# evfro/polara

Measured on NVIDIA H100. Metric: user-item pairs scored/sec (fused top-k) at rank 50, higher is better.
Workload: dtype f32 (bf16 tensor-core filter, exact fp32 rescoring)

## Files before the change

polara_b200/csrc/topk_tc.cu:

```cuda
#include <cuda_bf16.h>
#include <cfloat>
#include <cstdlib>
#include <cub/device/device_radix_sort.cuh>

#include "topk_common.cuh"

namespace {

constexpr int BM = 128;
constexpr int BN = 128;
constexpr int NCONS = 256;
constexpr int NTHREADS = NCONS + 32;
constexpr int CAPS = 16;
constexpr int MAX_STAGES = 10;
constexpr uint32_t STAGE_BYTES = BN * 128;
constexpr int PROBE_ITEMS = 256;
constexpr int HEAD_TILES = 8;
constexpr int HEAD_WORDS = HEAD_TILES * BN / 32;
constexpr long long SPIN_LIMIT_CYCLES = 4000000000ll;

struct TcParams {
    const __nv_bfloat16* Ap;
    const __nv_bfloat16* Bp;
    const float* E; int64_t lde;
// ... 161 lines not shown
    int64_t total = user_tiles * BM * chunks;
    if (gid >= total) return;
    int64_t tile = gid / ((int64_t)BM * chunks);
    int rem = (int)(gid % ((int64_t)BM * chunks));
    int row = rem / chunks, ch = rem % chunks;
    const int64_t tr = tile * BM + row;
    const int64_t u = (tr < m && uperm) ? (int64_t)__ldg(uperm + tr) : tr;
    __align__(16) __nv_bfloat16 out[8];
    uint32_t thr = 0;
    if (ch == rs / 8) {
        if (u < m) {
            thr = pack_threshold(t0[u]);
        } else {
            thr = 0x00007F7Fu;
        }
    }
#pragma unroll
    for (int j = 0; j < 8; ++j) {
        int kk = ch * 8 + j;
        float x = 0.f;
        if (u < m && kk < r) x = -__ldg(E + u * lde + kk);
        out[j] = __float2bfloat16_rn(x);
        if (kk == rs) out[j] = __ushort_as_bfloat16((unsigned short)(thr & 0xFFFFu));
        if (kk == rs + 1) out[j] = __ushort_as_bfloat16((unsigned short)(thr >> 16));
        if (kk == rs + 2 && u < m)
            out[j] = __ushort_as_bfloat16((unsigned short)(0x8000u | bf16_ceil_pos_bits(0.0079345703125f * enorm[u] + 1e-30f)));
    }
    size_t byte = (size_t)tile * BM * chunks * 16 + tile_byte(BM, row, ch * 8);
    *reinterpret_cast<uint4*>(reinterpret_cast<unsigned char*>(Ap) + byte) = *reinterpret_cast<const uint4*>(out);
}

__global__ void row_norm_kernel(const float* __restrict__ X, int64_t ld, int64_t rows, int r, float* __restrict__ norms,
                                float* __restrict__ max_out) {
    int64_t w = ((int64_t)blockIdx.x * blockDim.x + threadIdx.x) >> 5;
    int lane = threadIdx.x & 31;
    if (w >= rows) return;
    float s = 0.f;
    for (int t = lane; t < r; t += 32) { float x = __ldg(X + w * ld + t); s = fmaf(x, x, s); }
#pragma unroll
    for (int o = 16; o > 0; o >>= 1) s += __shfl_xor_sync(0xffffffffu, s, o);
    s = sqrtf(s) * 1.0001f;
    if (lane == 0) {
        if (norms) norms[w] = s;
        if (max_out) atomicMax(reinterpret_cast<int*>(max_out), __float_as_int(s));
    }
}

__global__ void iota_i32_kernel(int32_t* __restrict__ x, int64_t n) {
    int64_t i = (int64_t)blockIdx.x * blockDim.x + threadIdx.x;
    if (i < n) x[i] = (int32_t)i;
}

__global__ void invert_perm_kernel(const int32_t* __restrict__ perm, int64_t n, int32_t* __restrict__ inv) {
    int64_t i = (int64_t)blockIdx.x * blockDim.x + threadIdx.x;
    if (i < n) inv[perm[i]] = (int32_t)i;
}

__global__ void head_items_kernel(const int32_t* __restrict__ perm, int64_t n_head, uint32_t* __restrict__ in_head) {
    int64_t i = (int64_t)blockIdx.x * blockDim.x + threadIdx.x;
    if (i < n_head) { const int32_t item = perm[i]; atomicOr(in_head + (item >> 5), 1u << (item & 31)); }
}

__global__ void __launch_bounds__(256)
head_bitmap_kernel(const int64_t* __restrict__ seen_indptr, const int32_t* __restrict__ seen_indices,
                   int64_t seen_offset, const int32_t* __restrict__ inv_perm, const uint32_t* __restrict__ in_head,
                   int64_t m, int64_t n, uint32_t* __restrict__ bits) {
    static_assert(HEAD_WORDS == 32, "one bitmap word per lane");
    __shared__ uint32_t sw[8][HEAD_WORDS];
    const int64_t u = ((int64_t)blockIdx.x * blockDim.x + threadIdx.x) >> 5;
    const int lane = threadIdx.x & 31, warp = threadIdx.x >> 5;
    if (u >= m) return;
    sw[warp][lane] = 0u;
    __syncwarp();
    for (int64_t p = seen_indptr[u] + lane; p < seen_indptr[u + 1]; p += 32) {
        int64_t item = (int64_t)__ldg(seen_indices + p) - seen_offset;
        if (item < 0 || item >= n) continue;
        if (!((__ldg(in_head + (item >> 5)) >> (item & 31)) & 1u)) continue;
        int pos = __ldg(inv_perm + item);
        atomicOr(&sw[warp][pos >> 5], 0x80000000u >> (pos & 31));
    }
    __syncwarp();
    bits[u * HEAD_WORDS + lane] = sw[warp][lane];
}

__device__ __forceinline__ int first_cut_tile(float en, float t, const float* __restrict__ vnorm_sorted, int lo, int hi) {
    if (!(t > 0.f && t < CUDART_INF_F)) return hi;
    while (lo < hi) {
        const int mid = (lo + hi) >> 1;
        if (en * __ldg(vnorm_sorted + (int64_t)mid * BN) < t) hi = mid; else lo = mid + 1;
    }
    return lo;
}

__global__ void user_need_kernel(const float* __restrict__ enorm, const float* __restrict__ t0,
                                 const float* __restrict__ vnorm_sorted, int64_t m, int item_tiles, int32_t* __restrict__ need) {
    const int64_t u = (int64_t)blockIdx.x * blockDim.x + threadIdx.x;
    if (u < m) need[u] = first_cut_tile(__ldg(enorm + u), __ldg(t0 + u), vnorm_sorted, 0, item_tiles);
}

constexpr int PTU = 64, PTI = 128, PKS = 32;
constexpr int PNU = 2;
template <int PI>
struct ProbeSmem {
    float es[PKS][PTU + 4];
    float vs[PKS][PTI + 4];
    float sc[PTU][PI + 4];
    unsigned long long cand[8][PNU][32];
    float t0s[PTU];
};

__device__ __forceinline__ uint32_t ord_of(float x) {
    const uint32_t b = __float_as_uint(x);
    return (b & 0x80000000u) ? ~b : (b | 0x80000000u);
}
__device__ __forceinline__ float ord_to_float(uint32_t o) {
    return __uint_as_float((o & 0x80000000u) ? (o & 0x7FFFFFFFu) : ~o);
}

template <int PL>
__device__ __noinline__ void probe_select_rounds(unsigned long long (&key)[PL], int lane, int k,
                                                 pb200_cand* __restrict__ out, float* __restrict__ t0_u) {
    static_assert(PL == 8, "the sorting network below is for 8 keys per lane");
#define PB_CAS(A, B) { const unsigned long long x_ = key[A], y_ = key[B]; const bool g_ = x_ > y_; key[A] = g_ ? x_ : y_; key[B] = g_ ? y_ : x_; }
    PB_CAS(0, 1) PB_CAS(2, 3) PB_CAS(4, 5) PB_CAS(6, 7)
    PB_CAS(0, 2) PB_CAS(1, 3) PB_CAS(4, 6) PB_CAS(5, 7)
    PB_CAS(1, 2) PB_CAS(5, 6)
    PB_CAS(0, 4) PB_CAS(1, 5) PB_CAS(2, 6) PB_CAS(3, 7)
    PB_CAS(2, 4) PB_CAS(3, 5)
    PB_CAS(1, 2) PB_CAS(3, 4) PB_CAS(5, 6)
#undef PB_CAS
    float kth = -CUDART_INF_F;
    int produced = 0;
    pb200_cand mine; mine.score = -CUDART_INF_F; mine.id = -1;
    for (; produced < k; ++produced) {
        const uint32_t hh = (uint32_t)(key[0] >> 32), hl = (uint32_t)key[0];
        const uint32_t wh = __reduce_max_sync(0xffffffffu, hh);
        if (wh == 0u) break;
        const uint32_t wl = __reduce_max_sync(0xffffffffu, hh == wh ? hl : 0u);
        if (hh == wh && hl == wl) {
#pragma unroll
            for (int j = 0; j + 1 < PL; ++j) key[j] = key[j + 1];
            key[PL - 1] = 0ull;
        }
        const float ws = ord_to_float(wh);
        if (lane == (produced & 31)) { mine.score = ws; mine.id = (int)(0xFFFFFFFFu - wl); }
        if ((produced & 31) == 31) out[(produced - 31) + lane] = mine;
        kth = ws;
    }
    if (lane < (produced & 31)) out[(produced & ~31) + lane] = mine;
    for (int j = produced + lane; j < k; j += 32) { pb200_cand c; c.score = -CUDART_INF_F; c.id = -1; out[j] = c; }
    if (lane == 0) *t0_u = produced == k ? kth : -CUDART_INF_F;
}

template <int PI>
__global__ void __launch_bounds__(256)
probe_kernel(const float* __restrict__ E, int64_t lde, const float* __restrict__ V, int64_t ldv,
             const int32_t* __restrict__ perm, int64_t m, int64_t n_probe, int r, int k,
             const uint32_t* __restrict__ headbits, float* __restrict__ t0, pb200_cand* __restrict__ out_list,
             float* __restrict__ enorm, const float* __restrict__ vnorm_sorted, int item_tiles, int32_t* __restrict__ need) {
    extern __shared__ __align__(16) unsigned char praw[];
    ProbeSmem<PI>& sm = *reinterpret_cast<ProbeSmem<PI>*>(praw);
    const int tid = threadIdx.x, lane = tid & 31, warp = tid >> 5, tx = tid & 15, ty = tid >> 4;
    const int64_t u0 = (int64_t)blockIdx.x * PTU;
    const bool vec = ((lde | ldv) & 3) == 0 && ((reinterpret_cast<uintptr_t>(E) | reinterpret_cast<uintptr_t>(V)) & 15) == 0;
    const int n_ktiles = (r + PKS - 1) / PKS, n_tiles = (PI / PTI) * n_ktiles;
    const int64_t eu = u0 + (tid & (PTU - 1));
    const float* erow = eu < m ? E + eu * lde : nullptr;
    const float* vrow = nullptr;
    float4 pe[2], pv[4];
    auto fetch = [&](int tile) {
        const int i0 = (tile / n_ktiles) * PTI, k0 = (tile % n_ktiles) * PKS;
        if (tile % n_ktiles == 0) {
            const int64_t vpos = i0 + (tid & (PTI - 1));
            vrow = vpos < n_probe ? V + (int64_t)__ldg(perm + vpos) * ldv : nullptr;
        }
#pragma unroll
        for (int it = 0; it < 2; ++it) {
            const int kq = k0 + 4 * ((tid >> 6) + 4 * it);
            pe[it] = (erow && kq < r) ? __ldg(reinterpret_cast<const float4*>(erow + kq)) : make_float4(0.f, 0.f, 0.f, 0.f);
        }
#pragma unroll
        for (int it = 0; it < 4; ++it) {
            const int kq = k0 + 4 * ((tid >> 7) + 2 * it);
            pv[it] = (vrow && kq < r) ? __ldg(reinterpret_cast<const float4*>(vrow + kq)) : make_float4(0.f, 0.f, 0.f, 0.f);
        }
    };
    auto stash = [&](int tile) {
        const int k0 = (tile % n_ktiles) * PKS;
#pragma unroll
        for (int it = 0; it < 2; ++it) {
            const int q = (tid >> 6) + 4 * it, kq = k0 + 4 * q, row = tid & (PTU - 1);
            sm.es[4 * q + 0][row] = pe[it].x;
            sm.es[4 * q + 1][row] = kq + 1 < r ? pe[it].y : 0.f;
            sm.es[4 * q + 2][row] = kq + 2 < r ? pe[it].z : 0.f;
            sm.es[4 * q + 3][row] = kq + 3 < r ? pe[it].w : 0.f;
        }
#pragma unroll
        for (int it = 0; it < 4; ++it) {
            const int q = (tid >> 7) + 2 * it, kq = k0 + 4 * q, row = tid & (PTI - 1);
            sm.vs[4 * q + 0][row] = pv[it].x;
            sm.vs[4 * q + 1][row] = kq + 1 < r ? pv[it].y : 0.f;
            sm.vs[4 * q + 2][row] = kq + 2 < r ? pv[it].z : 0.f;
            sm.vs[4 * q + 3][row] = kq + 3 < r ? pv[it].w : 0.f;
        }
    };
    if (vec) fetch(0);
    float acc[4][8];
    float en2 = 0.f;
    for (int tile = 0; tile < n_tiles; ++tile) {
        const int i0 = (tile / n_ktiles) * PTI, k0 = (tile % n_ktiles) * PKS;
        if (k0 == 0) {
#pragma unroll
            for (int a = 0; a < 4; ++a)
#pragma unroll
                for (int b = 0; b < 8; ++b) acc[a][b] = 0.f;
        }
        if (vec) {
            stash(tile);
        } else {
#pragma unroll
            for (int it = 0; it < 8; ++it) {
                int e = tid + it * 256, row = e >> 5, kk = e & 31;
                int64_t u = u0 + row;
                sm.es[kk][row] = (u < m && k0 + kk < r) ? __ldg(E + u * lde + k0 + kk) : 0.f;
            }
#pragma unroll
            for (int it = 0; it < 16; ++it) {
                int e = tid + it * 256, row = e >> 5, kk = e & 31;
                int64_t pos = i0 + row;
                sm.vs[kk][row] = (pos < n_probe && k0 + kk < r) ? __ldg(V + (int64_t)__ldg(perm + pos) * ldv + k0 + kk) : 0.f;
            }
        }
        __syncthreads();
        if (vec && tile + 1 < n_tiles) fetch(tile + 1);
        const int kmax = min(PKS, r - k0);
        if (i0 == 0 && tid < PTU)
            for (int kk = 0; kk < kmax; ++kk) en2 = fmaf(sm.es[kk][tid], sm.es[kk][tid], en2);
        for (int kk = 0; kk < kmax; ++kk) {
            float4 e4 = *reinterpret_cast<const float4*>(&sm.es[kk][ty * 4]);
            float4 v0 = *reinterpret_cast<const float4*>(&sm.vs[kk][tx * 4]);
            float4 v1 = *reinterpret_cast<const float4*>(&sm.vs[kk][64 + tx * 4]);
            float a[4] = {e4.x, e4.y, e4.z, e4.w};
            float b[8] = {v0.x, v0.y, v0.z, v0.w, v1.x, v1.y, v1.z, v1.w};
#pragma unroll
            for (int i = 0; i < 4; ++i)
#pragma unroll
                for (int j = 0; j < 8; ++j) acc[i][j] = fmaf(a[i], b[j], acc[i][j]);
        }
        if (k0 + PKS >= r) {
#pragma unroll
            for (int i = 0; i < 4; ++i)
#pragma unroll
                for (int hseg = 0; hseg < 2; ++hseg) {
                    const int pos = i0 + 64 * hseg + tx * 4;
                    float4 x;
                    x.x = pos + 0 < n_probe ? acc[i][4 * hseg + 0] : -CUDART_INF_F;
                    x.y = pos + 1 < n_probe ? acc[i][4 * hseg + 1] : -CUDART_INF_F;
                    x.z = pos + 2 < n_probe ? acc[i][4 * hseg + 2] : -CUDART_INF_F;
                    x.w = pos + 3 < n_probe ? acc[i][4 * hseg + 3] : -CUDART_INF_F;
                    *reinterpret_cast<float4*>(&sm.sc[ty * 4 + i][pos]) = x;
                }
        }
        __syncthreads();
    }
    constexpr int PL = PI / 32;
    const uint32_t lt_mask = (1u << lane) - 1u;
    for (int ul = warp; ul < PTU; ul += 8 * PNU) {
        int64_t u[PNU];
        bool act[PNU];
        uint32_t seen_w[PNU], ord[PNU][PL], lmax[PNU], tau[PNU];
        int count[PNU] = {};
#pragma unroll
        for (int a = 0; a < PNU; ++a) {
            u[a] = u0 + ul + 8 * a;
            act[a] = ul + 8 * a < PTU && u[a] < m;
            seen_w[a] = 0u;
            if (act[a] && headbits && lane < PL) seen_w[a] = __ldg(headbits + u[a] * HEAD_WORDS + lane);
        }
#pragma unroll
        for (int a = 0; a < PNU; ++a) {
            lmax[a] = 0u;
#pragma unroll
            for (int j = 0; j < PL; ++j) {
                const int pos = lane + 32 * j;
                const uint32_t w = __shfl_sync(0xffffffffu, seen_w[a], j);
                const bool ok = act[a] && pos < n_probe && !(w & (0x80000000u >> lane));
                ord[a][j] = ok ? ord_of(sm.sc[act[a] ? ul + 8 * a : 0][pos] + 0.f) : 0u;
                lmax[a] = max(lmax[a], ord[a][j]);
            }
        }
        const bool small_k = k <= 32;
        if (small_k) {
            uint32_t rest[PNU], w[PNU];
#pragma unroll
            for (int a = 0; a < PNU; ++a) { rest[a] = lmax[a]; w[a] = 0u; }
            for (int i = 0; i < k; ++i) {
#pragma unroll
                for (int a = 0; a < PNU; ++a) {
                    w[a] = __reduce_max_sync(0xffffffffu, rest[a]);
                    if (rest[a] == w[a]) rest[a] = 0u;
                }
            }
#pragma unroll
            for (int a = 0; a < PNU; ++a) tau[a] = w[a] == 0u ? 1u : w[a];
#pragma unroll
            for (int a = 0; a < PNU; ++a) count[a] = 0;
#pragma unroll
            for (int j = 0; j < PL; ++j)
#pragma unroll
                for (int a = 0; a < PNU; ++a) {
                    const bool in = ord[a][j] >= tau[a];
                    const uint32_t b = __ballot_sync(0xffffffffu, in);
                    const int slot = count[a] + __popc(b & lt_mask);
                    if (in && slot < 32) sm.cand[warp][a][slot] = ((unsigned long long)ord[a][j] << 32) | (uint32_t)(lane + 32 * j);
                    count[a] += __popc(b);
                }
        }
        bool fast[PNU];
#pragma unroll
        for (int a = 0; a < PNU; ++a) fast[a] = act[a] && small_k && count[a] <= 32;
        __syncwarp();
        unsigned long long mine[PNU];
        uint32_t mpos[PNU];
#pragma unroll
        for (int a = 0; a < PNU; ++a) {
            mine[a] = 0ull;
            mpos[a] = 0u;
            if (fast[a] && lane < count[a]) {
                const unsigned long long c = sm.cand[warp][a][lane];
                mpos[a] = (uint32_t)c;
                const uint32_t id = (uint32_t)__ldg(perm + (uint32_t)c);
                mine[a] = (c & 0xFFFFFFFF00000000ull) | (unsigned long long)(0xFFFFFFFFu - id);
            }
        }
        __syncwarp();
#pragma unroll
        for (int a = 0; a < PNU; ++a) if (fast[a]) sm.cand[warp][a][lane] = mine[a];
        __syncwarp();
#pragma unroll
        for (int a = 0; a < PNU; ++a) {
            if (!fast[a]) continue;
            pb200_cand* out = out_list + u[a] * k;
            int rank = 0;
            for (int t = 0; t < count[a]; ++t) rank += sm.cand[warp][a][t] > mine[a] ? 1 : 0;
            if (lane < count[a] && rank < k) {
                pb200_cand c; c.score = ord_to_float((uint32_t)(mine[a] >> 32)); c.id = (int)(0xFFFFFFFFu - (uint32_t)mine[a]);
                if (c.score == 0.f) c.score = sm.sc[ul + 8 * a][mpos[a]];
                out[rank] = c;
                if (rank == k - 1) sm.t0s[ul + 8 * a] = c.score;
            }
            if (count[a] < k) {
                if (lane >= count[a] && lane < k) { pb200_cand c; c.score = -CUDART_INF_F; c.id = -1; out[lane] = c; }
                if (lane == 0) sm.t0s[ul + 8 * a] = -CUDART_INF_F;
            }
        }
        __syncwarp();
#pragma unroll
        for (int a = 0; a < PNU; ++a) {
            if (!act[a] || fast[a]) continue;
            unsigned long long key[PL];
#pragma unroll
            for (int j = 0; j < PL; ++j) {
                const uint32_t id = ord[a][j] ? (uint32_t)__ldg(perm + lane + 32 * j) : 0u;
                key[j] = ord[a][j] ? (((unsigned long long)ord[a][j] << 32) | (unsigned long long)(0xFFFFFFFFu - id)) : 0ull;
            }
            probe_select_rounds<PL>(key, lane, k, out_list + u[a] * k, &sm.t0s[ul + 8 * a]);
        }
        __syncwarp();
#pragma unroll
        for (int a = 0; a < PNU; ++a) {
            if (!act[a] || fast[a]) continue;
            pb200_cand* out = out_list + u[a] * k;
            for (int j = lane; j < k; j += 32) {
                const pb200_cand c = out[j];
                if (c.id >= 0 && c.score == 0.f) out[j].score = exact_score(E + u[a] * lde, V + (int64_t)c.id * ldv, r);
            }
        }
    }
    __syncthreads();
    if (tid < PTU && u0 + tid < m) {
        const int64_t uu = u0 + tid;
        const float t = sm.t0s[tid], en = sqrtf(en2) * 1.0001f;
        t0[uu] = t;
        enorm[uu] = en;
        if (need) need[uu] = first_cut_tile(en, t, vnorm_sorted, 0, item_tiles);
    }
}

__device__ __forceinline__ float exact_score_vec(const float* __restrict__ erow, const float* __restrict__ vrow, int r, bool vec_ok) {
    if (!vec_ok) return exact_score(erow, vrow, r);
    const int r4 = r / 4;
    const float4* e4 = reinterpret_cast<const float4*>(erow);
    const float4* v4 = reinterpret_cast<const float4*>(vrow);
    float s = 0.f;
    int t = 0;
    for (; t + 8 <= r4; t += 8) {
        float4 a[8], b[8];
#pragma unroll
        for (int i = 0; i < 8; ++i) { a[i] = __ldg(e4 + t + i); b[i] = __ldg(v4 + t + i); }
#pragma unroll
        for (int i = 0; i < 8; ++i) {
            s = fmaf(a[i].x, b[i].x, s); s = fmaf(a[i].y, b[i].y, s);
            s = fmaf(a[i].z, b[i].z, s); s = fmaf(a[i].w, b[i].w, s);
        }
    }
    for (; t + 4 <= r4; t += 4) {
        float4 a[4], b[4];
#pragma unroll
        for (int i = 0; i < 4; ++i) { a[i] = __ldg(e4 + t + i); b[i] = __ldg(v4 + t + i); }
#pragma unroll
        for (int i = 0; i < 4; ++i) {
            s = fmaf(a[i].x, b[i].x, s); s = fmaf(a[i].y, b[i].y, s);
            s = fmaf(a[i].z, b[i].z, s); s = fmaf(a[i].w, b[i].w, s);
        }
    }
    for (; t < r4; ++t) {
        float4 a = __ldg(e4 + t), b = __ldg(v4 + t);
        s = fmaf(a.x, b.x, s); s = fmaf(a.y, b.y, s); s = fmaf(a.z, b.z, s); s = fmaf(a.w, b.w, s);
    }
    for (int tt = r4 * 4; tt < r; ++tt) s = fmaf(__ldg(erow + tt), __ldg(vrow + tt), s);
    return s;
}

struct ListState {
    pb200_cand* list;
    int cnt;
    float kth;
};

__device__ __forceinline__ void list_insert(ListState& ls, int k, float s, int id) {
    if (ls.cnt == k) {
        pb200_cand last = ls.list[k - 1];
        if (!cand_before(s, id, last.score, last.id)) return;
    }
    int i = ls.cnt < k ? ls.cnt : k - 1;
    while (i > 0) {
        pb200_cand p = ls.list[i - 1];
        if (!cand_before(s, id, p.score, p.id)) break;
        ls.list[i] = p;
        --i;
    }
    pb200_cand c; c.score = s; c.id = id;
    ls.list[i] = c;
    if (ls.cnt < k) ls.cnt++;
    if (ls.cnt == k) ls.kth = ls.list[k - 1].score;
}

constexpr int COOP_MIN = 64;
struct CoopArgs {
    const float* V; int64_t ldv; const int32_t* perm; const int32_t* seen_indices; int64_t seen_offset; int64_t n; int r, k;
};
__device__ __noinline__ int coop_flush_row(const CoopArgs p, const float* __restrict__ erow, const uint2* __restrict__ stage_row,
                                           int n_entries, int64_t t_lo, int64_t sb, int64_t se, bool head_masked,
                                           pb200_cand* __restrict__ list, float t_row, bool vec_ok, int lane, int& cnt, float& kth) {
    int n_scored = 0;
    for (int e = 0; e < n_entries; ++e) {
        const uint2 ent = stage_row[e * 256];
        const int64_t pos = (int64_t)(t_lo + (ent.x >> 2)) * BN + (ent.x & 3) * 32 + lane;
        bool ok = ((ent.y << lane) & 0x80000000u) != 0u && pos < p.n;
        int item = -1;
        float s = 0.f;
        if (ok) {
            item = __ldg(p.perm + pos);
            if (sb < se && (!head_masked || pos >= HEAD_TILES * BN) &&
                seen_lookup(p.seen_indices, sb, se, (int)(item + p.seen_offset))) ok = false;
        }
        if (ok) {
            s = exact_score_vec(erow, p.V + (int64_t)item * p.ldv, p.r, vec_ok);
            ++n_scored;
            ok = !(s < t_row);
        }
        uint32_t pass = __ballot_sync(0xffffffffu, ok);
        while (pass) {
            const int l = __ffs(pass) - 1;
            pass &= pass - 1;
            const float sl = __shfl_sync(0xffffffffu, s, l);
            const int il = __shfl_sync(0xffffffffu, item, l);
            if (sl < t_row) continue;
            cnt = warp_list_insert(list, p.k, cnt, sl, il, lane);
            if (cnt == p.k) { kth = list[p.k - 1].score; t_row = fmaxf(t_row, kth); }
        }
    }
    return n_scored;
}

__global__ void __launch_bounds__(NTHREADS, 1)
score_topk_tc_kernel(const TcParams p) {
    extern __shared__ __align__(1024) unsigned char smem[];
    unsigned char* sA = smem + ((1024u - (smem_u32(smem) & 1023u)) & 1023u);
    unsigned char* sB = sA + p.a_bytes;
    uint2* sStage = reinterpret_cast<uint2*>(sB + (size_t)p.stages * STAGE_BYTES);
    volatile uint2* sThr = reinterpret_cast<volatile uint2*>(sStage + CAPS * 256);
    uint64_t* bars = reinterpret_cast<uint64_t*>(const_cast<uint2*>(sThr) + 256);
    const uint32_t bar_full = smem_u32(bars), bar_empty = smem_u32(bars + MAX_STAGES);
    const uint32_t bar_afull = smem_u32(bars + 2 * MAX_STAGES), bar_aempty = smem_u32(bars + 2 * MAX_STAGES + 1);
    volatile uint32_t* flush_gen = reinterpret_cast<volatile uint32_t*>(bars + 2 * MAX_STAGES + 2);
    volatile unsigned long long* sCut = reinterpret_cast<volatile unsigned long long*>(bars + 2 * MAX_STAGES + 4);
    volatile uint32_t* sStop = reinterpret_cast<volatile uint32_t*>(bars + 2 * MAX_STAGES + 4 + NCONS / 32);

    const int tid = threadIdx.x, warp = tid >> 5, lane = tid & 31;
    if (tid < 256) { const_cast<uint2*>(sThr)[tid] = make_uint2(0u, 0u); }
    if (tid < NCONS / 32) sCut[tid] = 0ull;
    if (tid < MAX_STAGES) sStop[tid] = 0u;
    if (tid == 0) {
        *flush_gen = 0u;
        for (int s = 0; s < p.stages; ++s) { mbar_init(bar_full + 8 * s, 1); mbar_init(bar_empty + 8 * s, NCONS / 32); }
        mbar_init(bar_afull, 1);
        mbar_init(bar_aempty, NCONS / 32);
        fence_barrier_init();
        if (p.hdbg && blockIdx.x == 0) p.hdbg[5] = bar_full;
    }
    __syncthreads();

    const int64_t n_groups = p.user_tiles * p.parts;
    const int64_t n_ctas = gridDim.x, cta = blockIdx.x;
    WorkItem wk;
    const uint32_t S = (uint32_t)p.stages;
    const int KA = (p.KP + 63) / 64;

    if (warp == NCONS / 32) {
        if (lane == 0) {
            uint32_t stage = 0, phase = 0, awork = 0;
            for (int64_t wi = 0; next_work(p, wi, cta, n_ctas, n_groups, wk); ++wi, ++awork) {
                const int64_t t_lo = min(p.item_tiles, p.tile_first + (int64_t)wk.part * p.tiles_per_part);
                int64_t t_hi = min(p.item_tiles, p.tile_first + (int64_t)(wk.part + 1) * p.tiles_per_part);
                if (p.need_sorted) t_hi = min(t_hi, max(t_lo, (int64_t)__ldg(p.need_sorted + wk.g * BM)));
                mbar_wait(bar_aempty, (awork & 1) ^ 1, p.stats, p.hdbg);
                mbar_arrive_expect_tx(bar_afull, p.a_bytes);
                bulk_g2s(smem_u32(sA), reinterpret_cast<const unsigned char*>(p.Ap) + (size_t)wk.g * p.a_bytes, p.a_bytes, bar_afull);
                for (int64_t t = t_lo; t < t_hi; ++t) {
                    if (p.need_sorted) {
                        bool all = true;
                        int64_t live_cut = 0;
#pragma unroll
                        for (int w = 0; w < NCONS / 32; ++w) {
                            const unsigned long long e = sCut[w];
                            all = all && (uint32_t)e == awork + 1;
                            live_cut = max(live_cut, (int64_t)(e >> 32));
// ... 133 lines not shown
                const int64_t t = t_lo + j;
                if (p.need_sorted) {
                    const uint32_t st = gslab % S, ph = (gslab / S) & 1u;
                    mbar_wait(bar_full + 8 * st, ph, p.stats, p.hdbg);
                    if (sStop[st]) {
                        ++gslab;
                        __syncwarp();
                        if (lane == 0) mbar_arrive(bar_empty + 8 * st);
                        break;
                    }
                }
                float d[64];
#pragma unroll
                for (int i = 0; i < 64; ++i) d[i] = 0.f;
                uint32_t prev = 0;
                for (int sl = 0; sl < KA; ++sl) {
                    const uint32_t st = gslab % S, ph = (gslab / S) & 1u;
                    ++gslab;
                    mbar_wait(bar_full + 8 * st, ph, p.stats, p.hdbg);
                    wg_fence_acc(d);
                    wg_fence();
#pragma unroll
                    for (int ks = 0; ks < 4; ++ks)
                        wgmma_m64n128k16(d, adesc0 + (uint64_t)((uint32_t)sl * (BM * 128 / 16) + (uint32_t)ks * 2),
                                         bdesc0 + (uint64_t)(st * (STAGE_BYTES / 16) + (uint32_t)ks * 2), (sl | ks) != 0);
                    wg_commit();
                    wg_fence_acc(d);
                    if (sl > 0) {
                        wg_wait<1>();
                        __syncwarp();
                        if (lane == 0) mbar_arrive(bar_empty + 8 * prev);
                    }
                    prev = st;
                }
                wg_wait<0>();
                wg_fence_acc(d);
                __syncwarp();
                if (lane == 0) mbar_arrive(bar_empty + 8 * prev);

                uint32_t w[2][4];
#pragma unroll
                for (int a = 0; a < 2; ++a)
#pragma unroll
                    for (int c = 0; c < 4; ++c) {
                        uint32_t mk = 0;
#pragma unroll
                        for (int i = 0; i < 4; ++i)
#pragma unroll
                            for (int b = 0; b < 2; ++b)
                                mk |= (__float_as_uint(d[4 * (4 * c + i) + 2 * a + b]) >> 31) << (31 - 8 * i - b);
                        mk >>= 2 * q;
                        mk |= __shfl_xor_sync(0xffffffffu, mk, 1);
                        mk |= __shfl_xor_sync(0xffffffffu, mk, 2);
                        w[a][c] = mk;
                    }
                const bool hi_row = (q >> 1) != 0;
                uint32_t m0 = hi_row ? (h ? w[1][2] : w[1][0]) : (h ? w[0][2] : w[0][0]);
                uint32_t m1 = hi_row ? (h ? w[1][3] : w[1][1]) : (h ? w[0][3] : w[0][1]);
                if (head && t < HEAD_TILES) {
                    const uint2 hb = __ldg(reinterpret_cast<const uint2*>(head + (int)t * (BN / 32) + 2 * h));
                    m0 &= ~hb.x; m1 &= ~hb.y;
                }
                const uint32_t code = (uint32_t)j << 2;
                if (m0 && live) { sStage[scount * 256 + etid] = make_uint2(code | (uint32_t)(2 * h), m0); ++scount; }
                if (m1 && live) { sStage[scount * 256 + etid] = make_uint2(code | (uint32_t)(2 * h + 1), m1); ++scount; }
                {
                    const uint32_t gen = *flush_gen;
                    const bool need = __any_sync(0xffffffffu, scount > CAPS - 2 || (scount >= 4 && t_row == -CUDART_INF_F));
                    if (need || gen != my_gen) {
                        if (need && gen == my_gen && lane == 0) atomicAdd(const_cast<uint32_t*>(flush_gen), 1u);
                        flush();
                        my_gen = *flush_gen;
                        if (p.need_sorted) publish_cut(t + 1);
                    }
                }
            }
            n_swept += (unsigned long long)j;
            flush();
            __syncwarp();
            if (lane == 0) mbar_arrive(bar_aempty);
        }
        if (p.stats && n_rescored) atomicAdd(p.stats + 1, n_rescored);
        if (p.stats && tid == 0 && n_swept) atomicAdd(p.stats + 5, n_swept);
    }
    __syncthreads();
}

}

int pb_score_tc(pb200_ctx* ctx, const float* E, int64_t lde, const float* V, int64_t ldv, int64_t m, int64_t n,
                int r, const int64_t* seen_indptr, const int32_t* seen_indices, int64_t seen_offset, int k,
                int* parts_out, pb200_cand** lists_out, Scratch& sc) {
    const int rs = (r + 1) & ~1;
    const int KP = ((rs + 3) + 15) / 16 * 16;
    const int KA = (KP + 63) / 64;
    const uint32_t a_bytes = BM * KA * 128, b_bytes = BN * KA * 128;
    const size_t fixed = (size_t)a_bytes + CAPS * 256 * sizeof(uint2) + 256 * sizeof(uint2) + (2 * MAX_STAGES + 4) * 8 +
                         (NCONS / 32) * 8 + MAX_STAGES * 4 + 1024;
    int dev_smem = 0;
    PB_CUDA(ctx, cudaDeviceGetAttribute(&dev_smem, cudaDevAttrMaxSharedMemoryPerBlockOptin, ctx->device));
    const int64_t user_tiles = ceil_div64(m, BM), item_tiles = ceil_div64(n, BN);
    const int stages = (int)std::min<int64_t>(MAX_STAGES, ((int64_t)dev_smem - (int64_t)fixed) / STAGE_BYTES);
    if (stages < 2) {
        ctx->err = "tensor-core scoring kernel: rank too large for the shared-memory pipeline (use the simt kernel)";
        return PB200_ENOTIMPL;
    }
    const int64_t n_probe = std::min<int64_t>(PROBE_ITEMS, (n / BN) * BN);
    const int64_t tile_first = n_probe / BN, sweep_tiles = item_tiles - tile_first;
    int parts = (int)std::max<int64_t>(1, std::min<int64_t>(std::min<int64_t>(ceil_div64(2 * (int64_t)ctx->num_sms, user_tiles), 64),
                                                              std::max<int64_t>(sweep_tiles, 1)));
    const int64_t tiles_per_part = std::max<int64_t>(1, ceil_div64(sweep_tiles, parts));
    parts = (int)std::max<int64_t>(1, ceil_div64(sweep_tiles, tiles_per_part));

    __nv_bfloat16 *Ap = nullptr, *Bp = nullptr;
    float *enorm = nullptr, *vnorm = nullptr, *vnorm_sorted = nullptr, *t0 = nullptr;
    int32_t *iota = nullptr, *perm = nullptr, *inv_perm = nullptr;
    uint32_t* headbits = nullptr;
    pb200_cand* lists = nullptr;
    PB_TRY(sc.alloc(&Ap, (size_t)user_tiles * BM * KA * 64));
    PB_TRY(sc.alloc(&Bp, (size_t)item_tiles * BN * KA * 64));
    PB_TRY(sc.alloc(&enorm, (size_t)m));
    PB_TRY(sc.alloc(&vnorm, (size_t)n));
    PB_TRY(sc.alloc(&vnorm_sorted, (size_t)n));
    PB_TRY(sc.alloc(&iota, (size_t)n));
    PB_TRY(sc.alloc(&perm, (size_t)n));
    PB_TRY(sc.alloc(&t0, (size_t)m));
    PB_TRY(sc.alloc(&lists, (size_t)(parts * 2 + 1) * m * k));

    row_norm_kernel<<<(unsigned)ceil_div64(n * 32, 256), 256, 0, ctx->stream>>>(V, ldv, n, r, vnorm, nullptr);
    iota_i32_kernel<<<(unsigned)ceil_div64(n, 256), 256, 0, ctx->stream>>>(iota, n);
    {
        size_t temp_bytes = 0;
        PB_CUDA(ctx, cub::DeviceRadixSort::SortPairsDescending(nullptr, temp_bytes, vnorm, vnorm_sorted, iota, perm, (int64_t)n, 0, 32, ctx->stream));
        uint8_t* temp = nullptr;
        PB_TRY(sc.alloc(&temp, temp_bytes));
        PB_CUDA(ctx, cub::DeviceRadixSort::SortPairsDescending(temp, temp_bytes, vnorm, vnorm_sorted, iota, perm, (int64_t)n, 0, 32, ctx->stream));
    }
    if (seen_indptr) {
        PB_TRY(sc.alloc(&inv_perm, (size_t)n));
        PB_TRY(sc.alloc(&headbits, (size_t)m * HEAD_WORDS));
        invert_perm_kernel<<<(unsigned)ceil_div64(n, 256), 256, 0, ctx->stream>>>(perm, n, inv_perm);
        uint32_t* in_head = nullptr;
        const int64_t n_head = std::min<int64_t>(n, (int64_t)HEAD_TILES * BN);
        PB_TRY(sc.alloc(&in_head, (size_t)ceil_div64(n, 32)));
        PB_CUDA(ctx, cudaMemsetAsync(in_head, 0, (size_t)ceil_div64(n, 32) * sizeof(uint32_t), ctx->stream));
        head_items_kernel<<<(unsigned)ceil_div64(n_head, 256), 256, 0, ctx->stream>>>(perm, n_head, in_head);
        head_bitmap_kernel<<<(unsigned)ceil_div64(m * 32, 256), 256, 0, ctx->stream>>>(seen_indptr, seen_indices, seen_offset,
                                                                                     inv_perm, in_head, m, n, headbits);
    }
    const bool prune = ctx->prune != 0;
    int32_t* need = nullptr;
    if (prune) PB_TRY(sc.alloc(&need, (size_t)m));
    {
        PB_CUDA(ctx, cudaFuncSetAttribute(probe_kernel<PROBE_ITEMS>, cudaFuncAttributeMaxDynamicSharedMemorySize, (int)sizeof(ProbeSmem<PROBE_ITEMS>)));
        probe_kernel<PROBE_ITEMS><<<(unsigned)ceil_div64(m, PTU), 256, sizeof(ProbeSmem<PROBE_ITEMS>), ctx->stream>>>(
            E, lde, V, ldv, perm, m, n_probe, r, k, headbits, t0, lists + (size_t)parts * 2 * m * k,
            enorm, vnorm_sorted, (int)item_tiles, ctx->bound_fn ? nullptr : need);
    }
    if (ctx->bound_fn) {
        const int st = ctx->bound_fn(ctx->bound_user, t0, m, PB200_F32);
        if (st != 0) {
            ctx->err = "bound hook failed with status " + std::to_string(st);
            return PB200_ECUDA;
        }
        if (prune) user_need_kernel<<<(unsigned)ceil_div64(m, 256), 256, 0, ctx->stream>>>(enorm, t0, vnorm_sorted, m, (int)item_tiles, need);
    }
    int32_t *uperm = nullptr, *need_sorted = nullptr;
    if (prune) {
        int32_t* uiota = nullptr;
        PB_TRY(sc.alloc(&uiota, (size_t)m));
        PB_TRY(sc.alloc(&uperm, (size_t)m));
        PB_TRY(sc.alloc(&need_sorted, (size_t)m));
        iota_i32_kernel<<<(unsigned)ceil_div64(m, 256), 256, 0, ctx->stream>>>(uiota, m);
        int end_bit = 1;
        while (end_bit < 31 && ((int64_t)1 << end_bit) <= item_tiles) ++end_bit;
        size_t temp_bytes = 0;
        PB_CUDA(ctx, cub::DeviceRadixSort::SortPairsDescending(nullptr, temp_bytes, need, need_sorted, uiota, uperm, m, 0, end_bit, ctx->stream));
        uint8_t* temp = nullptr;
        PB_TRY(sc.alloc(&temp, temp_bytes));
        PB_CUDA(ctx, cub::DeviceRadixSort::SortPairsDescending(temp, temp_bytes, need, need_sorted, uiota, uperm, m, 0, end_bit, ctx->stream));
    }
    {
        int64_t tot_b = item_tiles * BN * (KA * 8), tot_a = user_tiles * BM * (KA * 8);
        pack_items_kernel<<<(unsigned)ceil_div64(tot_b, 256), 256, 0, ctx->stream>>>(V, ldv, n, r, rs, KP, item_tiles, perm, vnorm_sorted, Bp);
        pack_users_kernel<<<(unsigned)ceil_div64(tot_a, 256), 256, 0, ctx->stream>>>(E, lde, m, r, rs, KP, user_tiles, uperm, enorm, t0, Ap);
    }
    if (sweep_tiles <= 0) {
        cudaEventRecord(ctx->ev0, ctx->stream);
        cudaEventRecord(ctx->ev1, ctx->stream);
        *parts_out = 1;
        *lists_out = lists + (size_t)parts * 2 * m * k;
        PB_CUDA(ctx, cudaGetLastError());
        return PB200_OK;
    }
    TcParams p;
    p.Ap = Ap; p.Bp = Bp; p.E = E; p.lde = lde; p.V = V; p.ldv = ldv; p.perm = perm; p.t0 = t0;
    p.m = m; p.n = n; p.r = r; p.KP = KP; p.rs = rs; p.k = k;
    p.user_tiles = user_tiles; p.item_tiles = item_tiles; p.parts = parts; p.tiles_per_part = tiles_per_part;
    p.tile_first = tile_first;
    p.seen_indptr = seen_indptr; p.seen_indices = seen_indices; p.seen_offset = seen_offset;
    p.lists = lists; p.stages = stages; p.a_bytes = a_bytes; p.b_bytes = b_bytes;
    p.uperm = uperm; p.need_sorted = need_sorted; p.enorm = enorm; p.vnorm_sorted = vnorm_sorted; p.headbits = headbits;
    p.stats = reinterpret_cast<unsigned long long*>(ctx->d_stats);
    p.hdbg = nullptr;
    if (ctx->h_dbg) {
        unsigned long long* dptr = nullptr;
        if (cudaHostGetDevicePointer(&dptr, ctx->h_dbg, 0) == cudaSuccess) p.hdbg = dptr;
    }
    const size_t smem_bytes = fixed + (size_t)stages * STAGE_BYTES;
    PB_CUDA(ctx, cudaFuncSetAttribute(score_topk_tc_kernel, cudaFuncAttributeMaxDynamicSharedMemorySize, (int)smem_bytes));
    const int64_t n_groups = user_tiles * parts;
    const unsigned grid = (unsigned)std::min<int64_t>(n_groups, ctx->num_sms);
    cudaEventRecord(ctx->ev0, ctx->stream);
    score_topk_tc_kernel<<<grid, NTHREADS, smem_bytes, ctx->stream>>>(p);
    cudaEventRecord(ctx->ev1, ctx->stream);
    ctx->stats[0] += (seen_indptr ? 13 : 10) + (prune ? 2 : 0) + (prune && ctx->bound_fn ? 1 : 0);
    ctx->stats[2] = (uint64_t)item_tiles; ctx->stats[3] = (uint64_t)user_tiles;
    ctx->stats[6] += (uint64_t)(user_tiles * sweep_tiles);
    PB_CUDA(ctx, cudaGetLastError());
    *parts_out = parts * 2 + 1;
    *lists_out = lists;
    return PB200_OK;
}
```

Before: 15330 billion.

## Add persistent probe kernel with smem-resident head items and double-buffered user rows

Adds a persistent probe kernel that loads the 256 head items' factor columns into shared memory once per CTA. It then loops over 32-user blocks, prefetching the next block's user rows and seen-bitmap words with cp.async double buffering. The old streamed probe kernel is kept as a fallback when shared memory does not allow two CTAs per SM, and the shared selection logic moves into a templated helper. The aim is to stop re-reading item vectors for every user tile and to hide load latency, at the cost of more shared memory per CTA. The probe is only one stage of the whole top-k pipeline.

```diff
diff --git a/polara_b200/csrc/topk_tc.cu b/polara_b200/csrc/topk_tc.cu
--- a/polara_b200/csrc/topk_tc.cu
+++ b/polara_b200/csrc/topk_tc.cu
@@ -337,9 +337,131 @@
     if (lane == 0) *t0_u = produced == k ? kth : -CUDART_INF_F;
 }
 
+template <int PI, int NU, typename IdOf, typename SeenOf>
+__device__ __forceinline__ void probe_select(const float (*sc)[PI + 4], unsigned long long (*cand)[PNU][32], float* t0s,
+                                             IdOf id_of, bool has_seen, SeenOf seen_word, int64_t u0, int64_t m,
+                                             int64_t n_probe, int k, pb200_cand* __restrict__ out_list,
+                                             const float* __restrict__ E, int64_t lde, const float* __restrict__ V,
+                                             int64_t ldv, int r, int warp, int lane) {
+    constexpr int PL = PI / 32;
+    const uint32_t lt_mask = (1u << lane) - 1u;
+    for (int ul = warp; ul < NU; ul += 8 * PNU) {
+        int64_t u[PNU];
+        bool act[PNU];
+        uint32_t seen_w[PNU], ord[PNU][PL], lmax[PNU], tau[PNU];
+        int count[PNU] = {};
+#pragma unroll
+        for (int a = 0; a < PNU; ++a) {
+            u[a] = u0 + ul + 8 * a;
+            act[a] = ul + 8 * a < NU && u[a] < m;
+            seen_w[a] = 0u;
+            if (act[a] && has_seen && lane < PL) seen_w[a] = seen_word(ul + 8 * a, lane);
+        }
+#pragma unroll
+        for (int a = 0; a < PNU; ++a) {
+            lmax[a] = 0u;
+#pragma unroll
+            for (int j = 0; j < PL; ++j) {
+                const int pos = lane + 32 * j;
+                const uint32_t w = __shfl_sync(0xffffffffu, seen_w[a], j);
+                const bool ok = act[a] && pos < n_probe && !(w & (0x80000000u >> lane));
+                ord[a][j] = ok ? ord_of(sc[act[a] ? ul + 8 * a : 0][pos] + 0.f) : 0u;
+                lmax[a] = max(lmax[a], ord[a][j]);
+            }
+        }
+        const bool small_k = k <= 32;
+        if (small_k) {
+            uint32_t rest[PNU], w[PNU];
+#pragma unroll
+            for (int a = 0; a < PNU; ++a) { rest[a] = lmax[a]; w[a] = 0u; }
+            for (int i = 0; i < k; ++i) {
+#pragma unroll
+                for (int a = 0; a < PNU; ++a) {
+                    w[a] = __reduce_max_sync(0xffffffffu, rest[a]);
+                    if (rest[a] == w[a]) rest[a] = 0u;
+                }
+            }
+#pragma unroll
+            for (int a = 0; a < PNU; ++a) tau[a] = w[a] == 0u ? 1u : w[a];
+#pragma unroll
+            for (int a = 0; a < PNU; ++a) count[a] = 0;
+#pragma unroll
+            for (int j = 0; j < PL; ++j)
+#pragma unroll
+                for (int a = 0; a < PNU; ++a) {
+                    const bool in = ord[a][j] >= tau[a];
+                    const uint32_t b = __ballot_sync(0xffffffffu, in);
+                    const int slot = count[a] + __popc(b & lt_mask);
+                    if (in && slot < 32) cand[warp][a][slot] = ((unsigned long long)ord[a][j] << 32) | (uint32_t)(lane + 32 * j);
+                    count[a] += __popc(b);
+                }
+        }
+        bool fast[PNU];
+#pragma unroll
+        for (int a = 0; a < PNU; ++a) fast[a] = act[a] && small_k && count[a] <= 32;
+        __syncwarp();
+        unsigned long long mine[PNU];
+        uint32_t mpos[PNU];
+#pragma unroll
+        for (int a = 0; a < PNU; ++a) {
+            mine[a] = 0ull;
+            mpos[a] = 0u;
+            if (fast[a] && lane < count[a]) {
+                const unsigned long long c = cand[warp][a][lane];
+                mpos[a] = (uint32_t)c;
+                const uint32_t id = (uint32_t)id_of((uint32_t)c);
+                mine[a] = (c & 0xFFFFFFFF00000000ull) | (unsigned long long)(0xFFFFFFFFu - id);
+            }
+        }
+        __syncwarp();
+#pragma unroll
+        for (int a = 0; a < PNU; ++a) if (fast[a]) cand[warp][a][lane] = mine[a];
+        __syncwarp();
+#pragma unroll
+        for (int a = 0; a < PNU; ++a) {
+            if (!fast[a]) continue;
+            pb200_cand* out = out_list + u[a] * k;
+            int rank = 0;
+            for (int t = 0; t < count[a]; ++t) rank += cand[warp][a][t] > mine[a] ? 1 : 0;
+            if (lane < count[a] && rank < k) {
+                pb200_cand c; c.score = ord_to_float((uint32_t)(mine[a] >> 32)); c.id = (int)(0xFFFFFFFFu - (uint32_t)mine[a]);
+                if (c.score == 0.f) c.score = sc[ul + 8 * a][mpos[a]];
+                out[rank] = c;
+                if (rank == k - 1) t0s[ul + 8 * a] = c.score;
+            }
+            if (count[a] < k) {
+                if (lane >= count[a] && lane < k) { pb200_cand c; c.score = -CUDART_INF_F; c.id = -1; out[lane] = c; }
+                if (lane == 0) t0s[ul + 8 * a] = -CUDART_INF_F;
+            }
+        }
+        __syncwarp();
+#pragma unroll
+        for (int a = 0; a < PNU; ++a) {
+            if (!act[a] || fast[a]) continue;
+            unsigned long long key[PL];
+#pragma unroll
+            for (int j = 0; j < PL; ++j) {
+                const uint32_t id = ord[a][j] ? (uint32_t)id_of(lane + 32 * j) : 0u;
+                key[j] = ord[a][j] ? (((unsigned long long)ord[a][j] << 32) | (unsigned long long)(0xFFFFFFFFu - id)) : 0ull;
+            }
+            probe_select_rounds<PL>(key, lane, k, out_list + u[a] * k, &t0s[ul + 8 * a]);
+        }
+        __syncwarp();
+#pragma unroll
+        for (int a = 0; a < PNU; ++a) {
+            if (!act[a] || fast[a]) continue;
+            pb200_cand* out = out_list + u[a] * k;
+            for (int j = lane; j < k; j += 32) {
+                const pb200_cand c = out[j];
+                if (c.id >= 0 && c.score == 0.f) out[j].score = exact_score(E + u[a] * lde, V + (int64_t)c.id * ldv, r);
+            }
+        }
+    }
+}
+
 template <int PI>
 __global__ void __launch_bounds__(256)
-probe_kernel(const float* __restrict__ E, int64_t lde, const float* __restrict__ V, int64_t ldv,
+probe_streamed_kernel(const float* __restrict__ E, int64_t lde, const float* __restrict__ V, int64_t ldv,
              const int32_t* __restrict__ perm, int64_t m, int64_t n_probe, int r, int k,
              const uint32_t* __restrict__ headbits, float* __restrict__ t0, pb200_cand* __restrict__ out_list,
              float* __restrict__ enorm, const float* __restrict__ vnorm_sorted, int item_tiles, int32_t* __restrict__ need) {
@@ -448,120 +570,9 @@
         }
         __syncthreads();
     }
-    constexpr int PL = PI / 32;
-    const uint32_t lt_mask = (1u << lane) - 1u;
-    for (int ul = warp; ul < PTU; ul += 8 * PNU) {
-        int64_t u[PNU];
-        bool act[PNU];
-        uint32_t seen_w[PNU], ord[PNU][PL], lmax[PNU], tau[PNU];
-        int count[PNU] = {};
-#pragma unroll
-        for (int a = 0; a < PNU; ++a) {
-            u[a] = u0 + ul + 8 * a;
-            act[a] = ul + 8 * a < PTU && u[a] < m;
-            seen_w[a] = 0u;
-            if (act[a] && headbits && lane < PL) seen_w[a] = __ldg(headbits + u[a] * HEAD_WORDS + lane);
-        }
-#pragma unroll
-        for (int a = 0; a < PNU; ++a) {
-            lmax[a] = 0u;
-#pragma unroll
-            for (int j = 0; j < PL; ++j) {
-                const int pos = lane + 32 * j;
-                const uint32_t w = __shfl_sync(0xffffffffu, seen_w[a], j);
-                const bool ok = act[a] && pos < n_probe && !(w & (0x80000000u >> lane));
-                ord[a][j] = ok ? ord_of(sm.sc[act[a] ? ul + 8 * a : 0][pos] + 0.f) : 0u;
-                lmax[a] = max(lmax[a], ord[a][j]);
-            }
-        }
-        const bool small_k = k <= 32;
-        if (small_k) {
-            uint32_t rest[PNU], w[PNU];
-#pragma unroll
-            for (int a = 0; a < PNU; ++a) { rest[a] = lmax[a]; w[a] = 0u; }
-            for (int i = 0; i < k; ++i) {
-#pragma unroll
-                for (int a = 0; a < PNU; ++a) {
-                    w[a] = __reduce_max_sync(0xffffffffu, rest[a]);
-                    if (rest[a] == w[a]) rest[a] = 0u;
-                }
-            }
-#pragma unroll
-            for (int a = 0; a < PNU; ++a) tau[a] = w[a] == 0u ? 1u : w[a];
-#pragma unroll
-            for (int a = 0; a < PNU; ++a) count[a] = 0;
-#pragma unroll
-            for (int j = 0; j < PL; ++j)
-#pragma unroll
-                for (int a = 0; a < PNU; ++a) {
-                    const bool in = ord[a][j] >= tau[a];
-                    const uint32_t b = __ballot_sync(0xffffffffu, in);
-                    const int slot = count[a] + __popc(b & lt_mask);
-                    if (in && slot < 32) sm.cand[warp][a][slot] = ((unsigned long long)ord[a][j] << 32) | (uint32_t)(lane + 32 * j);
-                    count[a] += __popc(b);
-                }
-        }
-        bool fast[PNU];
-#pragma unroll
-        for (int a = 0; a < PNU; ++a) fast[a] = act[a] && small_k && count[a] <= 32;
-        __syncwarp();
-        unsigned long long mine[PNU];
-        uint32_t mpos[PNU];
-#pragma unroll
-        for (int a = 0; a < PNU; ++a) {
-            mine[a] = 0ull;
-            mpos[a] = 0u;
-            if (fast[a] && lane < count[a]) {
-                const unsigned long long c = sm.cand[warp][a][lane];
-                mpos[a] = (uint32_t)c;
-                const uint32_t id = (uint32_t)__ldg(perm + (uint32_t)c);
-                mine[a] = (c & 0xFFFFFFFF00000000ull) | (unsigned long long)(0xFFFFFFFFu - id);
-            }
-        }
-        __syncwarp();
-#pragma unroll
-        for (int a = 0; a < PNU; ++a) if (fast[a]) sm.cand[warp][a][lane] = mine[a];
-        __syncwarp();
-#pragma unroll
-        for (int a = 0; a < PNU; ++a) {
-            if (!fast[a]) continue;
-            pb200_cand* out = out_list + u[a] * k;
-            int rank = 0;
-            for (int t = 0; t < count[a]; ++t) rank += sm.cand[warp][a][t] > mine[a] ? 1 : 0;
-            if (lane < count[a] && rank < k) {
-                pb200_cand c; c.score = ord_to_float((uint32_t)(mine[a] >> 32)); c.id = (int)(0xFFFFFFFFu - (uint32_t)mine[a]);
-                if (c.score == 0.f) c.score = sm.sc[ul + 8 * a][mpos[a]];
-                out[rank] = c;
-                if (rank == k - 1) sm.t0s[ul + 8 * a] = c.score;
-            }
-            if (count[a] < k) {
-                if (lane >= count[a] && lane < k) { pb200_cand c; c.score = -CUDART_INF_F; c.id = -1; out[lane] = c; }
-                if (lane == 0) sm.t0s[ul + 8 * a] = -CUDART_INF_F;
-            }
-        }
-        __syncwarp();
-#pragma unroll
-        for (int a = 0; a < PNU; ++a) {
-            if (!act[a] || fast[a]) continue;
-            unsigned long long key[PL];
-#pragma unroll
-            for (int j = 0; j < PL; ++j) {
-                const uint32_t id = ord[a][j] ? (uint32_t)__ldg(perm + lane + 32 * j) : 0u;
-                key[j] = ord[a][j] ? (((unsigned long long)ord[a][j] << 32) | (unsigned long long)(0xFFFFFFFFu - id)) : 0ull;
-            }
-            probe_select_rounds<PL>(key, lane, k, out_list + u[a] * k, &sm.t0s[ul + 8 * a]);
-        }
-        __syncwarp();
-#pragma unroll
-        for (int a = 0; a < PNU; ++a) {
-            if (!act[a] || fast[a]) continue;
-            pb200_cand* out = out_list + u[a] * k;
-            for (int j = lane; j < k; j += 32) {
-                const pb200_cand c = out[j];
-                if (c.id >= 0 && c.score == 0.f) out[j].score = exact_score(E + u[a] * lde, V + (int64_t)c.id * ldv, r);
-            }
-        }
-    }
+    probe_select<PI, PTU>(sm.sc, sm.cand, sm.t0s, [&](uint32_t pos) { return __ldg(perm + pos); }, headbits != nullptr,
+                          [&](int row, int j) { return __ldg(headbits + (u0 + row) * HEAD_WORDS + j); }, u0, m, n_probe, k,
+                          out_list, E, lde, V, ldv, r, warp, lane);
     __syncthreads();
     if (tid < PTU && u0 + tid < m) {
         const int64_t uu = u0 + tid;
@@ -569,6 +580,152 @@
         t0[uu] = t;
         enorm[uu] = en;
         if (need) need[uu] = first_cut_tile(en, t, vnorm_sorted, 0, item_tiles);
+    }
+}
+
+__device__ __forceinline__ void cp_async4(void* dst, const void* src) {
+    asm volatile("cp.async.ca.shared.global [%0], [%1], 4;" ::"r"(smem_u32(dst)), "l"(src) : "memory");
+}
+__device__ __forceinline__ void cp_async16(void* dst, const void* src) {
+    asm volatile("cp.async.cg.shared.global [%0], [%1], 16;" ::"r"(smem_u32(dst)), "l"(src) : "memory");
+}
+__device__ __forceinline__ void cp_async_commit() { asm volatile("cp.async.commit_group;" ::: "memory"); }
+__device__ __forceinline__ void cp_async_wait1() { asm volatile("cp.async.wait_group 1;" ::: "memory"); }
+
+constexpr int PRU = 32;
+template <int PI>
+struct ProbeResSmem {
+    float sc[PRU][PI + 4];
+    unsigned long long cand[8][PNU][32];
+    float t0s[PRU];
+    int32_t ids[PI];
+    uint32_t hb[2][PRU][PI / 32];
+};
+__host__ __device__ __forceinline__ int probe_res_stride(int r) {
+    const int se = (r + 3) & ~3;
+    return (se & 7) ? se : se + 4;
+}
+template <int PI>
+__host__ __device__ __forceinline__ size_t probe_res_smem_bytes(int r) {
+    return sizeof(ProbeResSmem<PI>) + sizeof(float) * ((size_t)2 * PRU * probe_res_stride(r) + (size_t)r * PI);
+}
+
+template <int PI>
+__global__ void __launch_bounds__(256, 2)
+probe_kernel(const float* __restrict__ E, int64_t lde, const float* __restrict__ V, int64_t ldv,
+             const int32_t* __restrict__ perm, int64_t m, int64_t n_probe, int r, int k,
+             const uint32_t* __restrict__ headbits, float* __restrict__ t0, pb200_cand* __restrict__ out_list,
+             float* __restrict__ enorm, const float* __restrict__ vnorm_sorted, int item_tiles, int32_t* __restrict__ need) {
+    static_assert(PI == 256, "one head item per thread in the load, two 128-item halves in the product");
+    extern __shared__ __align__(16) unsigned char praw[];
+    ProbeResSmem<PI>& sm = *reinterpret_cast<ProbeResSmem<PI>*>(praw);
+    const int SE = probe_res_stride(r);
+    float* const es = reinterpret_cast<float*>(praw + sizeof(ProbeResSmem<PI>));
+    float* const vs = es + 2 * PRU * SE;
+    const int tid = threadIdx.x, lane = tid & 31, warp = tid >> 5;
+    const bool vec = (lde & 3) == 0 && (reinterpret_cast<uintptr_t>(E) & 15) == 0;
+    const int64_t n_blocks = (m + PRU - 1) / PRU;
+    auto load_e = [&](int64_t b, int buf) {
+        float* dst = es + buf * PRU * SE;
+        const int64_t ub = b * PRU;
+        if (vec) {
+            const int q = (r + 3) >> 2;
+            for (int i = tid; i < PRU * q; i += 256) {
+                const int row = i / q, c = i - row * q;
+                if (ub + row < m) cp_async16(dst + row * SE + 4 * c, E + (ub + row) * lde + 4 * c);
+            }
+        } else {
+            for (int i = tid; i < PRU * r; i += 256) {
+                const int row = i / r, c = i - row * r;
+                if (ub + row < m) cp_async4(dst + row * SE + c, E + (ub + row) * lde + c);
+            }
+        }
+        if (headbits && tid < PRU * (PI / 128) && ub + tid / (PI / 128) < m) {
+            const int row = tid / (PI / 128), c = tid % (PI / 128);
+            cp_async16(&sm.hb[buf][row][4 * c], headbits + (ub + row) * HEAD_WORDS + 4 * c);
+        }
+        cp_async_commit();
+    };
+    int64_t b = blockIdx.x;
+    if (b < n_blocks) load_e(b, 0);
+    {
+        const int32_t id = tid < n_probe ? __ldg(perm + tid) : -1;
+        sm.ids[tid] = id < 0 ? 0 : id;
+        const float* vrow = V + (int64_t)(id < 0 ? 0 : id) * ldv;
+#pragma unroll 8
+        for (int kk = 0; kk < r; ++kk) vs[kk * PI + tid] = id >= 0 ? __ldg(vrow + kk) : 0.f;
+    }
+    const int h = warp & 1, ty = 2 * (warp >> 1) + (lane >> 4), tx = lane & 15;
+    const float* const vcol = vs + 128 * h + 4 * tx;
+    const int r4 = r & ~3;
+    for (int it = 0; b < n_blocks; b += gridDim.x, ++it) {
+        const int buf = it & 1;
+        if (b + gridDim.x < n_blocks) load_e(b + gridDim.x, buf ^ 1); else cp_async_commit();
+        cp_async_wait1();
+        __syncthreads();
+        const int64_t u0 = b * PRU;
+        const float* const eb = es + buf * PRU * SE;
+        float en2 = 0.f;
+        if (tid < PRU)
+            for (int kk = 0; kk < r; ++kk) en2 = fmaf(eb[tid * SE + kk], eb[tid * SE + kk], en2);
+        const float* const erow = eb + 4 * ty * SE;
+        float acc[4][8];
+#pragma unroll
+        for (int i = 0; i < 4; ++i)
+#pragma unroll
+            for (int j = 0; j < 8; ++j) acc[i][j] = 0.f;
+        for (int k0 = 0; k0 < r4; k0 += 4) {
+            float4 e4[4];
+#pragma unroll
+            for (int i = 0; i < 4; ++i) e4[i] = *reinterpret_cast<const float4*>(erow + i * SE + k0);
+#pragma unroll
+            for (int kk = 0; kk < 4; ++kk) {
+                const float4 v0 = *reinterpret_cast<const float4*>(vcol + (k0 + kk) * PI);
+                const float4 v1 = *reinterpret_cast<const float4*>(vcol + (k0 + kk) * PI + 64);
+                const float bv[8] = {v0.x, v0.y, v0.z, v0.w, v1.x, v1.y, v1.z, v1.w};
+#pragma unroll
+                for (int i = 0; i < 4; ++i) {
+                    const float a = kk == 0 ? e4[i].x : kk == 1 ? e4[i].y : kk == 2 ? e4[i].z : e4[i].w;
+#pragma unroll
+                    for (int j = 0; j < 8; ++j) acc[i][j] = fmaf(a, bv[j], acc[i][j]);
+                }
+            }
+        }
+        for (int kk = r4; kk < r; ++kk) {
+            const float4 v0 = *reinterpret_cast<const float4*>(vcol + kk * PI);
+            const float4 v1 = *reinterpret_cast<const float4*>(vcol + kk * PI + 64);
+            const float bv[8] = {v0.x, v0.y, v0.z, v0.w, v1.x, v1.y, v1.z, v1.w};
+#pragma unroll
+            for (int i = 0; i < 4; ++i) {
+                const float a = erow[i * SE + kk];
+#pragma unroll
+                for (int j = 0; j < 8; ++j) acc[i][j] = fmaf(a, bv[j], acc[i][j]);
+            }
+        }
+#pragma unroll
+        for (int i = 0; i < 4; ++i)
+#pragma unroll
+            for (int hseg = 0; hseg < 2; ++hseg) {
+                const int pos = 128 * h + 64 * hseg + tx * 4;
+                float4 x;
+                x.x = pos + 0 < n_probe ? acc[i][4 * hseg + 0] : -CUDART_INF_F;
+                x.y = pos + 1 < n_probe ? acc[i][4 * hseg + 1] : -CUDART_INF_F;
+                x.z = pos + 2 < n_probe ? acc[i][4 * hseg + 2] : -CUDART_INF_F;
+                x.w = pos + 3 < n_probe ? acc[i][4 * hseg + 3] : -CUDART_INF_F;
+                *reinterpret_cast<float4*>(&sm.sc[ty * 4 + i][pos]) = x;
+            }
+        __syncthreads();
+        probe_select<PI, PRU>(sm.sc, sm.cand, sm.t0s, [&](uint32_t pos) { return sm.ids[pos]; }, headbits != nullptr,
+                              [&](int row, int j) { return sm.hb[buf][row][j]; }, u0, m, n_probe, k, out_list, E, lde, V,
+                              ldv, r, warp, lane);
+        __syncthreads();
+        if (tid < PRU && u0 + tid < m) {
+            const int64_t uu = u0 + tid;
+            const float t = sm.t0s[tid], en = sqrtf(en2) * 1.0001f;
+            t0[uu] = t;
+            enorm[uu] = en;
+            if (need) need[uu] = first_cut_tile(en, t, vnorm_sorted, 0, item_tiles);
+        }
     }
 }
 
@@ -1008,10 +1165,24 @@
     int32_t* need = nullptr;
     if (prune) PB_TRY(sc.alloc(&need, (size_t)m));
     {
-        PB_CUDA(ctx, cudaFuncSetAttribute(probe_kernel<PROBE_ITEMS>, cudaFuncAttributeMaxDynamicSharedMemorySize, (int)sizeof(ProbeSmem<PROBE_ITEMS>)));
-        probe_kernel<PROBE_ITEMS><<<(unsigned)ceil_div64(m, PTU), 256, sizeof(ProbeSmem<PROBE_ITEMS>), ctx->stream>>>(
-            E, lde, V, ldv, perm, m, n_probe, r, k, headbits, t0, lists + (size_t)parts * 2 * m * k,
-            enorm, vnorm_sorted, (int)item_tiles, ctx->bound_fn ? nullptr : need);
+        const size_t res_bytes = probe_res_smem_bytes<PROBE_ITEMS>(r);
+        int res_ctas = 0;
+        if (res_bytes <= (size_t)dev_smem) {
+            PB_CUDA(ctx, cudaFuncSetAttribute(probe_kernel<PROBE_ITEMS>, cudaFuncAttributeMaxDynamicSharedMemorySize, (int)res_bytes));
+            PB_CUDA(ctx, cudaOccupancyMaxActiveBlocksPerMultiprocessor(&res_ctas, probe_kernel<PROBE_ITEMS>, 256, res_bytes));
+        }
+        pb200_cand* const probe_list = lists + (size_t)parts * 2 * m * k;
+        int32_t* const probe_need = ctx->bound_fn ? nullptr : need;
+        if (res_ctas >= 2) {
+            const int64_t grid = std::min<int64_t>(ceil_div64(m, PRU), (int64_t)res_ctas * ctx->num_sms);
+            probe_kernel<PROBE_ITEMS><<<(unsigned)grid, 256, res_bytes, ctx->stream>>>(
+                E, lde, V, ldv, perm, m, n_probe, r, k, headbits, t0, probe_list, enorm, vnorm_sorted, (int)item_tiles, probe_need);
+        } else {
+            PB_CUDA(ctx, cudaFuncSetAttribute(probe_streamed_kernel<PROBE_ITEMS>, cudaFuncAttributeMaxDynamicSharedMemorySize,
+                                              (int)sizeof(ProbeSmem<PROBE_ITEMS>)));
+            probe_streamed_kernel<PROBE_ITEMS><<<(unsigned)ceil_div64(m, PTU), 256, sizeof(ProbeSmem<PROBE_ITEMS>), ctx->stream>>>(
+                E, lde, V, ldv, perm, m, n_probe, r, k, headbits, t0, probe_list, enorm, vnorm_sorted, (int)item_tiles, probe_need);
+        }
     }
     if (ctx->bound_fn) {
         const int st = ctx->bound_fn(ctx->bound_user, t0, m, PB200_F32);
```

New measurement: 16060 billion (median of 6 runs). 1.05x the previous value.
